# ErickRosete/tacorl

Measured on AMD Instinct MI355X. Metric: offline grad-steps/sec (batch=256, 84x84 RGB), higher is better.
Workload: dtype bf16; 1 GPU; tacorl actor-critic training_step, frozen LMP (BASELINE configs[1]); per_gpu_batch=256, global_batch=256, window=16, image=84x84x3, frames=fp32 CHW (reference batch schema), latent_plan=16, n_action_samples=4, phase=Q (epoch>=bc_epochs), action_decoder_loss=every step (reference behaviour), parallelism=dp1, hip_graph=True, losses_finite=True

## Files before the change

### tacorl_amd/csrc/dense_ops.hip

```cpp
#include <stdio.h>
#include <stdlib.h>
#include <string.h>

#include <type_traits>

#include "../../include/tacorl_hip.h"
#include "enc_bwd_fused.h"
#include "mlp_fused.h"
#include "functors.h"

static thread_local char g_err[256] = "";
#define FAIL(code, ...)                        \
  do {                                         \
    snprintf(g_err, sizeof(g_err), __VA_ARGS__); \
    return (code);                             \
  } while (0)
#define CHECK(x)            \
  do {                      \
    int _r = (x);           \
    if (_r != TACORL_OK) return _r; \
  } while (0)

extern "C" const char* tacorl_hip_last_error(void) { return g_err; }
extern "C" int tacorl_hip_version(void) { return 1; }
// ... 737 lines not shown
  size_t scratch_bytes, fcwt_off[EBW_MAXP], fcwt_each, slab_off, slab_bytes, conv_off, total;
  long so[EBW_MAXP][6], ao[EBW_MAXP][5], sbase[EBW_MAXP];
  long maxn;
};
static const int kFcActs[2] = {ACT_RELU, ACT_NONE};
static bool enc_bwd_plan(int nprob, const int* n_img, int H, int W, EncBwdPlan& pl) {
  if (!enc_dims(H, W, pl.d) || !ebw_supported(H, W) || nprob < 1 || nprob > EBW_MAXP) return false;
  tacorl_encoder_param_layout(pl.po);
  long tot = 0;
  pl.maxn = 0;
  for (int p = 0; p < nprob; p++) {
    pl.sbase[p] = tot;
    tot += enc_bwd_scratch_layout(n_img[p], pl.d, pl.so[p]);
    tacorl_encoder_act_layout(n_img[p], H, W, pl.ao[p]);
    pl.maxn = n_img[p] > pl.maxn ? n_img[p] : pl.maxn;
  }
  size_t b = ((size_t)tot * sizeof(float) + 255) & ~(size_t)255;
  pl.scratch_bytes = b;
  pl.fcwt_each = (mlp_fused_wt_elems(2, kFcDims, nullptr) * 2 + 255) & ~(size_t)255;
  for (int p = 0; p < nprob; p++) { pl.fcwt_off[p] = b; b += pl.fcwt_each; }
  pl.slab_off = b;
  pl.slab_bytes = enc_fc_slab_bytes(nprob, pl.maxn);
  b += pl.slab_bytes;
  pl.conv_off = b;
  pl.total = b + ebw_ws_bytes(nprob, n_img, H, W);
  return true;
}
extern "C" size_t tacorl_encoder_bwd_fused_ws_bytes(int nprob, const int* n_img, int H, int W) {
  EncBwdPlan pl;
  return enc_bwd_plan(nprob, n_img, H, W, pl) ? pl.total : 0;
}
static void enc_bwd_conv_problems(int nprob, const void* const* img, const float* const* params, const float* const* act,
                                  float* const* grads, const int* n_img, const EncBwdPlan& pl, void* ws, EbwProblem* pr) {
  for (int p = 0; p < nprob; p++) {
    const float* P = params[p];
    float* G = grads ? grads[p] : nullptr;
    float* sc = (float*)ws + pl.sbase[p];
    pr[p].img = img ? img[p] : nullptr;
    pr[p].y1 = act ? act[p] + pl.ao[p][0] : nullptr; pr[p].y2 = act ? act[p] + pl.ao[p][1] : nullptr;
    pr[p].dz3 = sc + pl.so[p][2];
    pr[p].w2 = P + pl.po[E_W2]; pr[p].w3 = P + pl.po[E_W3];
    pr[p].g_w1 = G ? G + pl.po[E_W1] : nullptr; pr[p].g_b1 = G ? G + pl.po[E_B1] : nullptr;
    pr[p].g_w2 = G ? G + pl.po[E_W2] : nullptr; pr[p].g_b2 = G ? G + pl.po[E_B2] : nullptr;
    pr[p].g_w3 = G ? G + pl.po[E_W3] : nullptr; pr[p].g_b3 = G ? G + pl.po[E_B3] : nullptr;
    pr[p].n = n_img[p];
  }
}
static int enc_bwd_fc_chain(int nprob, const float* const* params, const float* const* act, const float* const* d_out,
                            const int* n_img, const EncBwdPlan& pl, void* ws, hipStream_t st, int mode) {
  long wo[2], bo[2], src[MF_MAXP * MF_MAXL], dzo[MF_MAXP * MF_MAXL];
  tacorl_mlp_param_layout(2, kFcDims, wo, bo);
  const float* fcp[EBW_MAXP];
  float *dz[EBW_MAXP], *dsa[EBW_MAXP];
  void* wt[EBW_MAXP];
  for (int p = 0; p < nprob; p++) {
    fcp[p] = params[p] + pl.po[E_FW1];
    src[p * MF_MAXL + 0] = pl.ao[p][4];
    src[p * MF_MAXL + 1] = -1;
    dzo[p * MF_MAXL + 0] = pl.sbase[p] + pl.so[p][0];
    dz[p] = (float*)ws;
    dsa[p] = (float*)ws + pl.sbase[p] + pl.so[p][1];
    wt[p] = (unsigned char*)ws + pl.fcwt_off[p];
  }
  return mlp_fused_bwd(nprob, fcp, act, d_out, 32, dz, dsa, 128, wt, n_img, 2, kFcDims, kFcActs, src, dzo, wo, st, mode);
}

extern "C" int tacorl_encoder_bwd_fused_pack(int nprob, const float* const* params, const int* n_img, int H, int W,
                                             void* ws, size_t ws_bytes, tacorl_stream_t stream) {
  EncBwdPlan pl;
  if (!enc_bwd_plan(nprob, n_img, H, W, pl)) FAIL(TACORL_EINVAL, "encoder_bwd_fused_pack: geometry %dx%d / nprob %d", H, W, nprob);
  if (ws_bytes < pl.total) FAIL(TACORL_ENOMEM, "encoder_bwd_fused_pack: workspace too small");
  EbwProblem pr[EBW_MAXP];
  enc_bwd_conv_problems(nprob, nullptr, params, nullptr, nullptr, n_img, pl, ws, pr);
  int rc = enc_bwd_fc_chain(nprob, params, nullptr, nullptr, n_img, pl, ws, (hipStream_t)stream, 1);
  if (rc == TACORL_OK) rc = ebw_conv_backward(nprob, pr, H, W, 0, (unsigned char*)ws + pl.conv_off, pl.total - pl.conv_off, (hipStream_t)stream, 1);
  if (rc != TACORL_OK) FAIL(rc, "encoder_bwd_fused_pack: launch failed (%d)", rc);
  return TACORL_OK;
}
extern "C" int tacorl_encoder_bwd_fused_head(int nprob, const float* const* params, const float* const* act,
                                             const float* const* d_out, const int* n_img, int H, int W, int prepacked,
                                             void* ws, size_t ws_bytes, tacorl_stream_t stream) {
  EncBwdPlan pl;
  if (!enc_bwd_plan(nprob, n_img, H, W, pl)) FAIL(TACORL_EINVAL, "encoder_bwd_fused_head: geometry %dx%d / nprob %d", H, W, nprob);
  if (ws_bytes < pl.total) FAIL(TACORL_ENOMEM, "encoder_bwd_fused_head: workspace too small");
  const int rc = enc_bwd_fc_chain(nprob, params, act, d_out, n_img, pl, ws, (hipStream_t)stream, prepacked ? 2 : 0);
  if (rc != TACORL_OK) FAIL(rc, "encoder_bwd_fused_head: launch failed (%d)", rc);
  return TACORL_OK;
}
extern "C" int tacorl_encoder_bwd_fused_fc_wgrad(int nprob, const float* const* act, const float* const* d_out,
                                                 float* const* grads, const int* n_img, int H, int W, int accumulate,
                                                 void* ws, size_t ws_bytes, tacorl_stream_t stream) {
  hipStream_t st = (hipStream_t)stream;
  EncBwdPlan pl;
  if (!enc_bwd_plan(nprob, n_img, H, W, pl)) FAIL(TACORL_EINVAL, "encoder_bwd_fused_fc_wgrad: geometry %dx%d / nprob %d", H, W, nprob);
  if (ws_bytes < pl.total) FAIL(TACORL_ENOMEM, "encoder_bwd_fused_fc_wgrad: workspace too small");
  const float *sa[EBW_MAXP], *h1[EBW_MAXP], *d_h1[EBW_MAXP];
  float *g_fw1[EBW_MAXP], *g_fb1[EBW_MAXP], *g_fw2[EBW_MAXP], *g_fb2[EBW_MAXP];
  for (int p = 0; p < nprob; p++) {
    sa[p] = act[p] + pl.ao[p][3]; h1[p] = act[p] + pl.ao[p][4];
    d_h1[p] = (const float*)ws + pl.sbase[p] + pl.so[p][0];
    float* G = grads[p];
    g_fw1[p] = G + pl.po[E_FW1]; g_fb1[p] = G + pl.po[E_FB1]; g_fw2[p] = G + pl.po[E_FW2]; g_fb2[p] = G + pl.po[E_FB2];
  }
  void* slab = (unsigned char*)ws + pl.slab_off;
  if (mlp_fused_wgrad_ok(nprob, 2, kFcDims) &&
      mlp_fused_wgrad_slab_floats(nprob, n_img, 2, kFcDims) * sizeof(float) <= pl.slab_bytes) {
    long yoffs[MF_MAXP * MF_MAXL] = {}, dzoffs[MF_MAXP * MF_MAXL] = {};
    const float* dzb[EBW_MAXP];
    for (int p = 0; p < nprob; p++) {
      yoffs[p * MF_MAXL] = pl.ao[p][4];
      dzoffs[p * MF_MAXL] = pl.sbase[p] + pl.so[p][0];
      dzb[p] = (const float*)ws;
    }
    const long wo[2] = {pl.po[E_FW1], pl.po[E_FW2]}, bo[2] = {pl.po[E_FB1], pl.po[E_FB2]};
    if (mlp_fused_wgrad(nprob, sa, 128, act, d_out, 32, dzb, grads, (float*)slab, n_img, 2, kFcDims, yoffs, dzoffs, wo, bo,
                        accumulate, st))
      FAIL(TACORL_ELAUNCH, "encoder_bwd_fused_fc_wgrad: launch failed");
    return TACORL_OK;
  }
  CHECK(k_linear_wgrad(nprob, h1, 256, d_out, 32, n_img, 256, 32, g_fw2, g_fb2, accumulate, slab, pl.slab_bytes, TACORL_BF16, st));
  CHECK(k_linear_wgrad(nprob, sa, 128, d_h1, 256, n_img, 128, 256, g_fw1, g_fb1, accumulate, slab, pl.slab_bytes, TACORL_BF16, st));
  return TACORL_OK;
}
extern "C" int tacorl_encoder_bwd_fused_conv(int nprob, const void* const* img, const float* const* params,
                                             const float* const* act, float* const* grads, const int* n_img, int H, int W,
                                             int accumulate, int prepacked, void* ws, size_t ws_bytes,
                                             tacorl_stream_t stream) {
  return tacorl_encoder_bwd_fused_conv_parts(nprob, img, params, act, grads, n_img, H, W, accumulate, prepacked, 127, ws,
                                             ws_bytes, stream);
}
extern "C" int tacorl_encoder_bwd_fused_conv_parts(int nprob, const void* const* img, const float* const* params,
                                                   const float* const* act, float* const* grads, const int* n_img, int H,
                                                   int W, int accumulate, int prepacked, int parts, void* ws,
                                                   size_t ws_bytes, tacorl_stream_t stream) {
  hipStream_t st = (hipStream_t)stream;
  EncBwdPlan pl;
  if (!enc_bwd_plan(nprob, n_img, H, W, pl)) FAIL(TACORL_EINVAL, "encoder_bwd_fused_conv: geometry %dx%d / nprob %d", H, W, nprob);
  if (ws_bytes < pl.total) FAIL(TACORL_ENOMEM, "encoder_bwd_fused_conv: workspace too small");
  if (pl.d.c3.OH * pl.d.c3.OW > 4 * SAB_MAXI_HUGE) FAIL(TACORL_EINVAL, "encoder_bwd_fused: conv3 output too large");
  if ((parts & EBW_ALL) && (parts & EBW_ALL) != EBW_ALL && !prepacked)
    FAIL(TACORL_EINVAL, "encoder_bwd_fused_conv_parts: partial calls need prepacked fragments");
  EbwProblem pr[EBW_MAXP];
  enc_bwd_conv_problems(nprob, img, params, act, grads, n_img, pl, ws, pr);
  SabArgs sb{};
  for (int p = 0; p < nprob; p++) {
    float* sc = (float*)ws + pl.sbase[p];
    sb.y3[p] = act[p] + pl.ao[p][2]; sb.temp[p] = params[p] + pl.po[E_T]; sb.sa[p] = act[p] + pl.ao[p][3];
    sb.d_sa[p] = sc + pl.so[p][1]; sb.dz3[p] = sc + pl.so[p][2]; sb.dtp[p] = sc + pl.so[p][5];
    sb.gtemp[p] = grads[p] + pl.po[E_T]; sb.n[p] = n_img[p];
  }
  const char* fe = getenv("TACORL_EBW_FUSE3");
  const int fuse3 = fe ? atoi(fe) : 1;
  const bool fused3 = fuse3 && (parts & 127) == 127 && ebw_fused3_supported(H, W);
  if (fused3) {
    for (int p = 0; p < nprob; p++) {
      pr[p].y3 = sb.y3[p]; pr[p].temp = sb.temp[p]; pr[p].sa = sb.sa[p]; pr[p].d_sa = sb.d_sa[p];
      pr[p].dtp = sb.dtp[p]; pr[p].g_temp = sb.gtemp[p];
    }
  }
  if (pl.maxn > 0 && (parts & 1) && !fused3) {
    const int P3 = pl.d.c3.OH * pl.d.c3.OW;
    if (P3 <= 4 * 13) hipLaunchKernelGGL(softargmax_bwd_batch_kernel<13>, dim3((unsigned)pl.maxn, nprob), dim3(256), 0, st, sb, P3, pl.d.c3.OW);
    else if (P3 <= 4 * SAB_MAXI_BIG) hipLaunchKernelGGL(softargmax_bwd_batch_kernel<SAB_MAXI_BIG>, dim3((unsigned)pl.maxn, nprob), dim3(256), 0, st, sb, P3, pl.d.c3.OW);
    else hipLaunchKernelGGL(softargmax_bwd_batch_kernel<SAB_MAXI_HUGE>, dim3((unsigned)pl.maxn, nprob), dim3(256), 0, st, sb, P3, pl.d.c3.OW);
    hipLaunchKernelGGL(sum_to_scalar_batch_kernel, dim3(nprob), dim3(256), 0, st, sb, accumulate);
  }
  if (!(parts & EBW_ALL)) return hipGetLastError() == hipSuccess ? TACORL_OK : TACORL_ELAUNCH;
  const int rc = ebw_conv_backward(nprob, pr, H, W, accumulate, (unsigned char*)ws + pl.conv_off, pl.total - pl.conv_off, st, prepacked ? 2 : 0,
                                   (parts & EBW_ALL) | (fused3 ? EBW_FUSED3 : 0));
  if (rc != TACORL_OK) FAIL(rc, "encoder_bwd_fused_conv: conv backward launch failed (%d)", rc);
  return hipGetLastError() == hipSuccess ? TACORL_OK : TACORL_ELAUNCH;
}
extern "C" int tacorl_encoder_bwd_fused(int nprob, const void* const* img, const float* const* params,
                                        const float* const* act, const float* const* d_out, float* const* grads,
                                        const int* n_img, int H, int W, int accumulate, void* ws, size_t ws_bytes,
                                        tacorl_stream_t stream) {
  int rc = tacorl_encoder_bwd_fused_head(nprob, params, act, d_out, n_img, H, W, 0, ws, ws_bytes, stream);
  if (rc == TACORL_OK) rc = tacorl_encoder_bwd_fused_fc_wgrad(nprob, act, d_out, grads, n_img, H, W, accumulate, ws, ws_bytes, stream);
  if (rc == TACORL_OK) rc = tacorl_encoder_bwd_fused_conv(nprob, img, params, act, grads, n_img, H, W, accumulate, 0, ws, ws_bytes, stream);
  return rc;
}

extern "C" long tacorl_mlp_param_layout(int L, const int* dims, long* w_off, long* b_off) {
  long off = 0;
  for (int l = 0; l < L; l++) {
    if (w_off) w_off[l] = off;
    off = al4(off + (long)dims[l + 1] * dims[l]);
    if (b_off) b_off[l] = off;
    off = al4(off + dims[l + 1]);
  }
  return off;
}
extern "C" long tacorl_mlp_act_layout(int M, int L, const int* dims, const int* acts, long* z_off, long* y_off) {
  long off = 0;
  for (int l = 0; l < L; l++) {
    if (z_off) z_off[l] = -1;
    if (acts[l] == ACT_SILU) { if (z_off) z_off[l] = off; off = al4(off + (long)M * dims[l + 1]); }
    if (y_off) y_off[l] = off;
    off = al4(off + (long)M * dims[l + 1]);
  }
  return off;
}
#define MLP_MAXL 8

struct OutActTbl { const float* d[GEMM_MAXP]; const float* y[GEMM_MAXP]; float* dz[GEMM_MAXP]; int M[GEMM_MAXP]; };
__global__ __launch_bounds__(256) void out_act_grad_kernel(OutActTbl t, int ldo, int N, int act) {
  const int p = blockIdx.y;
  const long total = (long)t.M[p] * N;
  for (long e = (long)blockIdx.x * 256 + threadIdx.x; e < total; e += (long)gridDim.x * 256) {
    const long m = e / N;
    t.dz[p][e] = t.d[p][m * ldo + (e - m * N)] * act_grad(act, t.y[p][e]);
  }
}
static int out_act_grad(int nprob, const OutActTbl& t, int ldo, int N, int act, hipStream_t st) {
  long mx = 0;
  for (int p = 0; p < nprob; p++) mx = (long)t.M[p] * N > mx ? (long)t.M[p] * N : mx;
  if (mx == 0) return TACORL_OK;
  const int gx = cdiv(mx, 256) > 1024 ? 1024 : cdiv(mx, 256);
  hipLaunchKernelGGL(out_act_grad_kernel, dim3(gx, nprob), dim3(256), 0, st, t, ldo, N, act);
  return hipGetLastError() == hipSuccess ? TACORL_OK : TACORL_ELAUNCH;
}

extern "C" int tacorl_mlp_fwd(int nprob, const float* const* x, int ldx, const float* const* params,
                              float* const* act, const int* M, int L, const int* dims, const int* acts, int cd,
                              tacorl_stream_t stream) {
  hipStream_t st = (hipStream_t)stream;
  if (L < 1 || L > MLP_MAXL || nprob < 1 || nprob > GEMM_MAXP) FAIL(TACORL_EINVAL, "mlp_fwd: bad L/nprob");
  long wo[MLP_MAXL], bo[MLP_MAXL];
  tacorl_mlp_param_layout(L, dims, wo, bo);
  for (int l = 0; l < L; l++) {
    const float *xin[GEMM_MAXP], *w[GEMM_MAXP], *b[GEMM_MAXP];
    float *y[GEMM_MAXP], *z[GEMM_MAXP];
    for (int p = 0; p < nprob; p++) {
      long zo[MLP_MAXL], yo[MLP_MAXL];
      tacorl_mlp_act_layout(M[p], L, dims, acts, zo, yo);
      xin[p] = l == 0 ? x[p] : act[p] + yo[l - 1];
      w[p] = params[p] + wo[l]; b[p] = params[p] + bo[l];
      y[p] = act[p] + yo[l]; z[p] = zo[l] >= 0 ? act[p] + zo[l] : nullptr;
    }
    CHECK(k_linear_fwd(nprob, xin, l == 0 ? ldx : dims[l], w, b, y, z, M, dims[l], dims[l + 1], dims[l + 1], acts[l], cd, st));
  }
  return TACORL_OK;
}

extern "C" int tacorl_mlp_fwd_fused_supported(int nprob, int L, const int* dims, int ldx) {
  return mlp_fused_fwd_ok(nprob, L, dims, ldx) ? 1 : 0;
}
extern "C" int tacorl_mlp_lean_supported(int nprob, int L, const int* dims, int ldx, int ldo, int ldd) {
  return mlp_fused_fwd_ok(nprob, L, dims, ldx) && mlp_fused_bwd_ok(nprob, L, dims, ldo, ldd) && mlp_fused_wgrad_ok(nprob, L, dims) ? 1 : 0;
}
static int mlp_fwd_fused_impl(int nprob, const float* const* x, int ldx, const float* const* params,
                              const void* const* params_bf16, float* const* act, const int* M, int L,
                              const int* dims, const int* acts, int lean, tacorl_stream_t stream, const MlpXGather* gather) {
  if (!mlp_fused_fwd_ok(nprob, L, dims, ldx)) FAIL(TACORL_EINVAL, "mlp_fwd_fused: shapes not supported");
  for (int p = 0; p < nprob; p++)
    if (!aligned16(params[p]) || ((uintptr_t)params_bf16[p] & 7) || (!gather && !aligned16(x[p])))
      FAIL(TACORL_EINVAL, "mlp_fwd_fused: problem %d: misaligned pointer", p);
  long wo[MLP_MAXL], bo[MLP_MAXL];
  tacorl_mlp_param_layout(L, dims, wo, bo);
  const float *xs[2][MF_MAXP], *ps[2][MF_MAXP];
  const void* pb[2][MF_MAXP];
  float* as[2][MF_MAXP];
  int Ms[2][MF_MAXP], gm[2][MF_MAXP], n[2] = {0, 0};
  long zo[MF_MAXP * MF_MAXL], yo[MF_MAXP * MF_MAXL], ybf[MF_MAXP * MF_MAXL], sbf[MF_MAXP * MF_MAXL], yout[MF_MAXP];
  for (int p = 0; p < nprob; p++) {
    long z1[MLP_MAXL], y1[MLP_MAXL];
    tacorl_mlp_act_layout(M[p], L, dims, acts, z1, y1);
    const int b = (lean && mlp_big_prob_ok(M[p], L, dims, acts)) ? 1 : 0, q = n[b]++;
    gm[b][q] = p;
    if (gather && gather->xb[p] && (!b || M[p] >= 16384 || !aligned16(gather->xb[p])))
      FAIL(TACORL_EINVAL, "mlp_fwd_fused_gather_xb: problem %d: the bf16 input rows are written only for a lean site's problems of "
                          "2048 .. 16383 rows, 16-byte aligned", p);
    xs[b][q] = x ? x[p] : nullptr; ps[b][q] = params[p]; pb[b][q] = params_bf16[p]; as[b][q] = act[p]; Ms[b][q] = M[p];
    for (int l = 0; l < L; l++) {
      if (b) { ybf[q * MF_MAXL + l] = y1[l]; sbf[q * MF_MAXL + l] = z1[l]; }
      else {
        zo[q * MF_MAXL + l] = z1[l];
        yo[q * MF_MAXL + l] = (lean && l + 1 < L && z1[l] >= 0) ? -1 : y1[l];
      }
    }
    if (b) yout[q] = y1[L - 1];
  }
  if (n[1]) {
    const int rc = mlp_big_fwd(n[1], xs[1], ldx, ps[1], pb[1], as[1], Ms[1], L, dims, acts, ybf, sbf, yout, wo, bo, (hipStream_t)stream, gather, gm[1]);
    if (rc != TACORL_OK) FAIL(rc, "mlp_fwd_fused: many-row launch failed (%d)", rc);
  }
  if (n[0]) {
    const int rc = mlp_fused_fwd(n[0], xs[0], ldx, ps[0], pb[0], as[0], Ms[0], L, dims, acts, zo, yo, wo, bo, (hipStream_t)stream, gather, gm[0]);
    if (rc != TACORL_OK) FAIL(rc, "mlp_fwd_fused: launch failed (%d)", rc);
  }
  return TACORL_OK;
}
extern "C" int tacorl_mlp_fwd_fused(int nprob, const float* const* x, int ldx, const float* const* params,
                                    const void* const* params_bf16, float* const* act, const int* M, int L,
                                    const int* dims, const int* acts, int lean, tacorl_stream_t stream) {
  return mlp_fwd_fused_impl(nprob, x, ldx, params, params_bf16, act, M, L, dims, acts, lean, stream, nullptr);
}
extern "C" int tacorl_mlp_fwd_fused_gather_supported(int nprob, const int* M, int L, const int* dims, const int* acts, int ldx,
                                                     int lean) {
  (void)M; (void)acts; (void)lean;
  return mlp_fused_fwd_ok(nprob, L, dims, ldx) ? 1 : 0;
}
namespace {
struct XbWritten { const void* ptr; int M; };
thread_local XbWritten g_xb_written[16];
thread_local int g_xb_next = 0;
void xb_note(const void* ptr, int M) {
  for (XbWritten& e : g_xb_written)
    if (e.ptr == ptr) { e.M = M; return; }
  g_xb_written[g_xb_next] = XbWritten{ptr, M};
  g_xb_next = (g_xb_next + 1) % 16;
}
bool xb_noted(const void* ptr, int M) {
  for (const XbWritten& e : g_xb_written)
    if (e.ptr == ptr && e.M == M) return true;
  return false;
}
void xb_forget(const void* ptr) {
  for (XbWritten& e : g_xb_written)
    if (e.ptr == ptr) e = XbWritten{nullptr, 0};
}
}
// ... 335 lines not shown
```

### tacorl_amd/csrc/enc_bwd_fused.h

```cpp
#pragma once
#include <hip/hip_runtime.h>
#include <stddef.h>

#define EBW_MAXP 8

struct EbwProblem {
  const void* img;
  const void* y1;
  const void* y2;
  const float* dz3;
  const float* w2;
  const float* w3;
  float *g_w1, *g_b1, *g_w2, *g_b2, *g_w3, *g_b3;
  int n;
  const float *y3, *temp, *sa, *d_sa;
  float *dtp, *g_temp;
};

bool ebw_supported(int H, int W);
size_t ebw_ws_bytes(int nprob, const int* n_img, int H, int W);
enum { EBW_DGRAD3 = 2, EBW_WGRAD3 = 4, EBW_DGRAD2 = 8, EBW_WGRAD2 = 16, EBW_WGRAD1 = 32, EBW_REDUCE = 64, EBW_ALL = 126,
       EBW_FUSED3 = 128 };
bool ebw_fused3_supported(int H, int W);
int ebw_conv_backward(int nprob, const EbwProblem* pr, int H, int W, int accumulate, void* ws, size_t ws_bytes,
                      hipStream_t st, int mode, int parts = EBW_ALL);
```

### tacorl_amd/csrc/encoder_bwd_fused.hip

```cpp
#include "enc_bwd_fused.h"

#include <stdlib.h>

#include <type_traits>

#include "common.h"

namespace {

constexpr int NT = 512;
constexpr int NW = NT / 64;

constexpr int cmax(int a, int b) { return a > b ? a : b; }
constexpr int pitch8(int need) { return (need % 16 <= 8) ? need - need % 16 + 8 : need - need % 16 + 24; }

template <int KH_, int S_, int CI_, int CO_, int IH_, int IW_>
struct ConvL {
  static constexpr int KH = KH_, KW = KH_, S = S_, CI = CI_, CO = CO_, IH = IH_, IW = IW_;
  static constexpr int OH = (IH - KH) / S + 1, OW = (IW - KW) / S + 1;
  static constexpr int PH = (IH + S - 1) / S, PW = (IW + S - 1) / S;
  static constexpr int KA = KH / S, KB = KW / S;
  static constexpr int TAPS = KH * KW * CI;
  static constexpr int NPL = CI * S * S;
  static constexpr int PWP = (PW + 7) / 8 * 8;
// ... 622 lines not shown
      float v[G::K3];
#pragma unroll
      for (int k = 0; k < G::K3; k++) v[k] = vn[k];
      const float gx = gn[0], gy = gn[1], dot = gn[0] * fn[0] + gn[1] * fn[1];
      asm volatile("" : : "v"(gx), "v"(gy), "v"(dot) : "memory");
#pragma unroll
      for (int k = 0; k < G::K3; k++) asm volatile("" : : "v"(v[k]) : "memory");
      if (nxt < n_img) { fetch(nxt); fetch3(nxt); }
      const __bf16* yb = y2s + kb * G::Y2E;
      float mx = -INFINITY;
#pragma unroll
      for (int k = 0; k < G::K3; k++) {
        v[k] *= it;
        if (wl + NW3 * k < G::P3) mx = fmaxf(mx, v[k]);
      }
      float se = 0.f;
#pragma unroll
      for (int k = 0; k < G::K3; k++) se += (wl + NW3 * k < G::P3) ? __expf(v[k] - mx) : 0.f;
      shm[wl * 64 + lane] = mx;
      shs[wl * 64 + lane] = se;
      __syncthreads();
      {
        float mw[NW3], sw[NW3];
#pragma unroll
        for (int ww = 0; ww < NW3; ww++) { mw[ww] = shm[ww * 64 + lane]; sw[ww] = shs[ww * 64 + lane]; }
        __builtin_amdgcn_sched_barrier(0);
#pragma unroll
        for (int ww = 0; ww < NW3; ww++) mx = fmaxf(mx, mw[ww]);
        se = 0.f;
#pragma unroll
        for (int ww = 0; ww < NW3; ww++) se += sw[ww] * __expf(mw[ww] - mx);
      }
      const float rse = 1.0f / se;
#pragma unroll
      for (int k = 0; k < G::K3; k++) {
        const int i = wl + NW3 * k;
        if (i < G::P3) {
          const int iy = i / L::OW;
          const float pr = __expf(v[k] - mx) * rse;
          const float ds = pr * (gx * (float)(i - iy * L::OW) + gy * (float)iy - dot);
          dt -= ds * v[k] * it;
          dzh[((iy + L::HA) * L::C + (i - iy * L::OW) + L::HB) * L::PP + lane] = (__bf16)(v[k] != 0.f ? ds * it : 0.f);
        }
      }
      if (img != j0) flush(img - a.wpp, z2s + (kb ^ 1) * G::Z2E);
      __syncthreads();
      if constexpr (ROLE == 0) {
        __bf16* zw = z2s + kb * G::Z2E;
#pragma unroll
        for (int tg = 0; tg < NGRP3; tg++) {
          f32x4 o[TG3];
#pragma unroll
          for (int u = 0; u < TG3; u++) o[u] = f32x4{0.f, 0.f, 0.f, 0.f};
          constexpr int HK = L::KS / 2;
          static_assert(L::KS % 2 == 0, "fragment steps in two halves");
          auto aoff = [&](int ks) {
            const int tp = ks / (L::CO / 32), hf = ks % (L::CO / 32), ta = tp / L::KB, tb = tp % L::KB;
            return ((L::HA - ta) * L::C + L::HB - tb) * L::PP + 32 * hf;
          };
          bf16x8 A[TG3][HK];
#pragma unroll
          for (int ks = 0; ks < HK; ks++)
#pragma unroll
            for (int u = 0; u < TG3; u++)
              A[u][ks] = *reinterpret_cast<const bf16x8*>(dzh + abase[tg * TG3 + u < MT ? tg * TG3 + u : MT - 1] + aoff(ks));
          __builtin_amdgcn_sched_barrier(0);
#pragma unroll
          for (int ks = 0; ks < L::KS; ks++) {
#pragma unroll
            for (int u = 0; u < TG3; u++) {
              o[u] = __builtin_amdgcn_mfma_f32_16x16x32_bf16(Bf[ks], A[u][ks % HK], o[u], 0, 0, 0);
              if (ks + HK < L::KS)
                A[u][ks % HK] = *reinterpret_cast<const bf16x8*>(dzh + abase[tg * TG3 + u < MT ? tg * TG3 + u : MT - 1] + aoff(ks + HK));
            }
            __builtin_amdgcn_sched_barrier(0);
          }
#pragma unroll
          for (int u = 0; u < TG3; u++) {
            const int t = tg * TG3 + u;
            if (t >= MT) continue;
            const int oi = obase + t * 16 * L::CI;
            if (oi < L::PH * L::PW * L::CI) {
              const uint2 yv = *reinterpret_cast<const uint2*>(yb + (oi >> 6) * G::CIP + (oi & 63));
              const bool m0 = (((yv.x & 0xffffu) - 1u) & 0xffffu) < 0x7fffu, m1 = (((yv.x >> 16) - 1u) & 0xffffu) < 0x7fffu;
              const bool m2 = (((yv.y & 0xffffu) - 1u) & 0xffffu) < 0x7fffu, m3 = (((yv.y >> 16) - 1u) & 0xffffu) < 0x7fffu;
              *reinterpret_cast<bf16x4*>(zw + oi) =
                  bf16x4{(__bf16)(m0 ? o[u][0] : 0.f), (__bf16)(m1 ? o[u][1] : 0.f), (__bf16)(m2 ? o[u][2] : 0.f),
                         (__bf16)(m3 ? o[u][3] : 0.f)};
            }
          }
        }
      } else {
#pragma unroll
        for (int s = 0; s < G::KS; s++) {
          constexpr int JB = (G::NPW + 2) / 3;
          bf16x8 A[G::MPW], B[JB];
#pragma unroll
          for (int i = 0; i < G::MPW; i++) {
            const int col = 16 * (mg * G::MPW + i) + 4 * pc;
            A[i] = tr_frag(dzh + zr0[s] + col, dzh + zr1[s] + col);
          }
#pragma unroll
          for (int jb = 0; jb < G::NPW; jb += JB) {
#pragma unroll
            for (int j = jb; j < jb + JB && j < G::NPW; j++) {
              const int tofs = ((j / L::KW) * L::IW + j % L::KW) * G::CIP;
              B[j - jb] = tr_frag(yb + ir0[s] + coff + tofs, yb + ir1[s] + coff + tofs);
            }
            __builtin_amdgcn_sched_barrier(0);
#pragma unroll
            for (int j = jb; j < jb + JB && j < G::NPW; j++)
#pragma unroll
              for (int i = 0; i < G::MPW; i++) acc[i][j] = __builtin_amdgcn_mfma_f32_16x16x32_bf16(A[i], B[j - jb], acc[i][j], 0, 0, 0);
            __builtin_amdgcn_sched_barrier(0);
          }
          if (ng == 0) {
#pragma unroll
            for (int i = 0; i < G::MPW; i++) bacc[i] = __builtin_amdgcn_mfma_f32_16x16x32_bf16(A[i], ones, bacc[i], 0, 0, 0);
          }
        }
      }
      if (nxt < n_img) put(y2s + (kb ^ 1) * G::Y2E);
      __syncthreads();
    }
    if (j0 < n_img) flush(j0 + ((n_img - 1 - j0) / a.wpp) * a.wpp, z2s + (kb ^ 1) * G::Z2E);
    if constexpr (ROLE == 1) {
      float* sl = a.slab + (long)blockIdx.x * TG::SLABF;
#pragma unroll
      for (int i = 0; i < G::MPW; i++)
#pragma unroll
        for (int j = 0; j < G::NPW; j++)
          *reinterpret_cast<f32x4*>(sl + (((wv * G::MPW + i) * G::NPW + j) * 64 + lane) * 4) = acc[i][j];
      if (ng == 0 && l16 == 0) {
#pragma unroll
        for (int i = 0; i < G::MPW; i++)
#pragma unroll
          for (int r = 0; r < 4; r++) sl[L::CO * L::TAPS + 16 * (mg * G::MPW + i) + 4 * g + r] = bacc[i][r];
      }
    }
    dt = wave_sum(dt);
    if (lane == 0) shd[w] = dt;
    __syncthreads();
    if (tid == 0 && j0 < n_img) {
      float sum = 0.f;
#pragma unroll
      for (int ww = 0; ww < NW3; ww++) sum += shd[ww];
      a.dtp[p][j0] = sum;
    }
  };
  if (w < ND3) run(std::integral_constant<int, 0>{});
  else run(std::integral_constant<int, 1>{});
}

inline size_t al256(size_t x) { return (x + 255) & ~(size_t)255; }
inline int cdivi(long a, long b) { return (int)((a + b - 1) / b); }
constexpr int cdivi_c(int a, int b) { return (a + b - 1) / b; }

struct WsPlan {
  size_t wpk2[EBW_MAXP], wpk3[EBW_MAXP], dz2[EBW_MAXP], dz1[EBW_MAXP], slab1, slab2, slab3, total;
  int wpp;
};
template <class G>
WsPlan plan(int nprob, const int* n) {
  WsPlan w{};
  long maxn = 1;
  for (int p = 0; p < nprob; p++) maxn = n[p] > maxn ? n[p] : maxn;
  const int per = 256 / nprob > 1 ? 256 / nprob : 1;
  w.wpp = (int)(per < maxn ? per : maxn);
  size_t off = 0;
  for (int p = 0; p < nprob; p++) {
    w.wpk2[p] = off; off += al256((size_t)G::L2::NCOMBO * G::L2::KS * 64 * 16);
    w.wpk3[p] = off; off += al256((size_t)G::L3::NCOMBO * G::L3::KS * 64 * 16);
    w.dz2[p] = off; off += al256((size_t)n[p] * G::L3::IH * G::L3::IW * 64 * 2);
    w.dz1[p] = off; off += al256((size_t)n[p] * G::L2::IH * G::L2::IW * 32 * 2);
  }
  const size_t nwg = (size_t)nprob * w.wpp;
  w.slab1 = off; off += al256(nwg * TrGeo<typename G::L1>::SLABF * 4);
  w.slab2 = off; off += al256(nwg * TrGeo<typename G::L2>::SLABF * 4);
  w.slab3 = off; off += al256(nwg * TrGeo<typename G::L3>::SLABF * 4);
  w.total = off;
  return w;
}

template <class K>
int set_lds(K kern, size_t bytes) {
  return hipFuncSetAttribute(reinterpret_cast<const void*>(kern), hipFuncAttributeMaxDynamicSharedMemorySize, (int)bytes) ==
                 hipSuccess ? 0 : -1;
}

template <class L, class InT, class DzT>
int launch_wgrad_tr(const WgArgs& a, int nwg, hipStream_t st) {
  auto kern = ebw_wgrad_tr_kernel<L, InT, DzT>;
  constexpr size_t lds = TrGeo<L>::lds_bytes;
  static int once = set_lds(kern, lds);
  if (once) return TACORL_ELAUNCH;
  hipLaunchKernelGGL(kern, dim3(nwg), dim3(NT), lds, st, a);
  return TACORL_OK;
}
template <class L, class DzT>
int launch_dgrad(const DgArgs& a, int nwg, hipStream_t st) {
  auto kern = ebw_dgrad_kernel<L, DzT>;
  constexpr size_t lds = dgrad_lds_bytes<L>();
  static int once = set_lds(kern, lds);
  if (once) return TACORL_ELAUNCH;
  hipLaunchKernelGGL(kern, dim3(nwg), dim3(NT), lds, st, a);
  return TACORL_OK;
}
template <class L>
int launch_l3(const L3Args& a, int nwg, hipStream_t st) {
  auto kern = ebw_l3_kernel<L>;
  constexpr size_t lds = L3Geo<L>::lds_bytes;
  static int once = set_lds(kern, lds);
  if (once) return TACORL_ELAUNCH;
  hipLaunchKernelGGL(kern, dim3(nwg), dim3(NT3), lds, st, a);
  return TACORL_OK;
}
template <class G>
int run(int nprob, const EbwProblem* pr, int accumulate, void* ws, size_t ws_bytes, hipStream_t st, int mode, int parts) {
  using L1 = typename G::L1; using L2 = typename G::L2; using L3 = typename G::L3;
  int n[EBW_MAXP];
  for (int p = 0; p < nprob; p++) n[p] = pr[p].n;
  const WsPlan w = plan<G>(nprob, n);
  if (ws_bytes < w.total) return TACORL_ENOMEM;
  unsigned char* base = (unsigned char*)ws;
  const int nwg = nprob * w.wpp;
  PkArgs k2{}, k3{};
  for (int p = 0; p < nprob; p++) {
    k2.w[p] = pr[p].w2; k2.out[p] = (uint4*)(base + w.wpk2[p]);
    k3.w[p] = pr[p].w3; k3.out[p] = (uint4*)(base + w.wpk3[p]);
  }
  if (mode != 2) {
    hipLaunchKernelGGL((ebw_pack2_kernel<L2, L3>), dim3(cdivi(L2::NCOMBO * L2::KS * 64, 256) + cdivi(L3::NCOMBO * L3::KS * 64, 256), nprob),
                       dim3(256), 0, st, k2, k3);
  }
  if (mode == 1) return hipGetLastError() == hipSuccess ? TACORL_OK : TACORL_ELAUNCH;
  DgArgs d3{}, d2{};
  WgArgs g3{}, g2{}, g1{};
  float *gw1[EBW_MAXP], *gb1[EBW_MAXP], *gw2[EBW_MAXP], *gb2[EBW_MAXP], *gw3[EBW_MAXP], *gb3[EBW_MAXP];
  for (int p = 0; p < nprob; p++) {
    __bf16* dz2 = (__bf16*)(base + w.dz2[p]);
    __bf16* dz1 = (__bf16*)(base + w.dz1[p]);
    d3.dz[p] = pr[p].dz3; d3.yin[p] = (const __bf16*)pr[p].y2; d3.wpk[p] = k3.out[p]; d3.dx[p] = dz2; d3.n[p] = n[p];
    d2.dz[p] = dz2; d2.yin[p] = (const __bf16*)pr[p].y1; d2.wpk[p] = k2.out[p]; d2.dx[p] = dz1; d2.n[p] = n[p];
    g3.in[p] = pr[p].y2; g3.dz[p] = pr[p].dz3; g3.n[p] = n[p];
    g2.in[p] = pr[p].y1; g2.dz[p] = dz2; g2.n[p] = n[p];
    g1.in[p] = pr[p].img; g1.dz[p] = dz1; g1.n[p] = n[p];
    gw1[p] = pr[p].g_w1; gb1[p] = pr[p].g_b1; gw2[p] = pr[p].g_w2; gb2[p] = pr[p].g_b2;
    gw3[p] = pr[p].g_w3; gb3[p] = pr[p].g_b3;
  }
  d3.wpp = d2.wpp = g3.wpp = g2.wpp = g1.wpp = w.wpp;
  constexpr int dg2 = 2;
  long maxn = 1;
  for (int p = 0; p < nprob; p++) maxn = n[p] > maxn ? n[p] : maxn;
  auto per_cu = [](size_t lds) { return (size_t)dg2 * lds <= 160 * 1024 ? dg2 : 1; };
  const int k3w = per_cu(dgrad_lds_bytes<L3>()), k2w = per_cu(dgrad_lds_bytes<L2>());
  d3.wpp = (int)((long)k3w * w.wpp < maxn ? (long)k3w * w.wpp : maxn);
  d2.wpp = (int)((long)k2w * w.wpp < maxn ? (long)k2w * w.wpp : maxn);
  g1.slab = (float*)(base + w.slab1); g2.slab = (float*)(base + w.slab2); g3.slab = (float*)(base + w.slab3);
  int rc;
  const bool fused3 = (parts & EBW_FUSED3) != 0;
  if (fused3 && (parts & EBW_ALL) != EBW_ALL) return TACORL_EINVAL;
  {
    if (fused3) {
      L3Args f{};
      for (int p = 0; p < nprob; p++) {
        f.y3[p] = pr[p].y3; f.temp[p] = pr[p].temp; f.sa[p] = pr[p].sa; f.d_sa[p] = pr[p].d_sa;
        f.y2[p] = (const __bf16*)pr[p].y2; f.wpk[p] = k3.out[p]; f.dz2[p] = (__bf16*)(base + w.dz2[p]);
        f.dtp[p] = pr[p].dtp; f.n[p] = n[p];
      }
      f.slab = g3.slab; f.wpp = w.wpp;
      if constexpr (L3Geo<L3>::ok) {
        if ((rc = launch_l3<L3>(f, nwg, st))) return rc;
      } else {
        return TACORL_EINVAL;
      }
    } else {
      if ((parts & EBW_DGRAD3) && (rc = launch_dgrad<L3, float>(d3, nprob * d3.wpp, st))) return rc;
      if ((parts & EBW_WGRAD3) && (rc = launch_wgrad_tr<L3, __bf16, float>(g3, nwg, st))) return rc;
    }
    if ((parts & EBW_DGRAD2) && (rc = launch_dgrad<L2, __bf16>(d2, nprob * d2.wpp, st))) return rc;
    if ((parts & EBW_WGRAD2) && (rc = launch_wgrad_tr<L2, __bf16, __bf16>(g2, nwg, st))) return rc;
    if ((parts & EBW_WGRAD1) && (rc = launch_wgrad_tr<L1, __bf16, __bf16>(g1, nwg, st))) return rc;
    if (!(parts & EBW_REDUCE)) return hipGetLastError() == hipSuccess ? TACORL_OK : TACORL_ELAUNCH;
    RdTrArgs t{};
    t.slab[0] = g1.slab; t.slab[1] = g2.slab; t.slab[2] = g3.slab;
    auto fill = [&](int l, auto geo, int co, int taps) {
      using TG = decltype(geo);
      t.co[l] = co; t.taps[l] = taps; t.mpw[l] = TG::MPW; t.npw[l] = TG::NPW; t.mgrp[l] = TG::T::MGRP;
      t.ngrp[l] = TG::T::NGRP; t.kgrp[l] = TG::T::KGRP; t.slabf[l] = TG::SLABF;
    };
    fill(0, TrGeo<L1>{}, L1::CO, L1::TAPS); fill(1, TrGeo<L2>{}, L2::CO, L2::TAPS); fill(2, TrGeo<L3>{}, L3::CO, L3::TAPS);
    t.wpp = w.wpp; t.accumulate = accumulate;
    for (int p = 0; p < nprob; p++) {
      t.gw[0][p] = gw1[p]; t.gb[0][p] = gb1[p]; t.gw[1][p] = gw2[p]; t.gb[1][p] = gb2[p];
      t.gw[2][p] = gw3[p]; t.gb[2][p] = gb3[p];
    }
    constexpr int maxper_t = cmax(L1::SLABF, cmax(L2::SLABF, L3::SLABF));
    static_assert(cdivi_c(maxper_t, 64) - 1 > cdivi_c(L1::SLABF, 64), "the temperature block must lie beyond conv1's elements");
    if (fused3) {
      for (int p = 0; p < nprob; p++) { t.dtp[p] = pr[p].dtp; t.g_temp[p] = pr[p].g_temp; t.ndt[p] = n[p] < w.wpp ? n[p] : w.wpp; }
      t.ileave[2] = 1; t.mpw[2] = L3Geo<L3>::MPW; t.npw[2] = L3Geo<L3>::NPW; t.mgrp[2] = L3Tile::MGRP; t.ngrp[2] = L3Tile::NGRP;
    }
    hipLaunchKernelGGL(ebw_reduce_tr_kernel, dim3(cdivi(maxper_t, 64), 3 * nprob), dim3(256), 0, st, t);
    return hipGetLastError() == hipSuccess ? TACORL_OK : TACORL_ELAUNCH;
  }
}

}

#define EBW_GEOMS(X) X(84, 84) X(64, 64) X(44, 60) X(128, 128) X(150, 200)

bool ebw_fused3_supported(int H, int W) {
#define X(h, w) if (H == h && W == w) return L3Geo<Geo<h, w>::L3>::ok;
  EBW_GEOMS(X)
#undef X
  return false;
}
bool ebw_supported(int H, int W) {
#define X(h, w) if (H == h && W == w) return true;
  EBW_GEOMS(X)
#undef X
  return false;
}
size_t ebw_ws_bytes(int nprob, const int* n_img, int H, int W) {
  if (nprob < 1 || nprob > EBW_MAXP) return 0;
#define X(h, w) if (H == h && W == w) return plan<Geo<h, w>>(nprob, n_img).total;
  EBW_GEOMS(X)
#undef X
  return 0;
}
int ebw_conv_backward(int nprob, const EbwProblem* pr, int H, int W, int accumulate, void* ws, size_t ws_bytes,
                      hipStream_t st, int mode, int parts) {
  if (nprob < 1 || nprob > EBW_MAXP) return TACORL_EINVAL;
#define X(h, w) if (H == h && W == w) return run<Geo<h, w>>(nprob, pr, accumulate, ws, ws_bytes, st, mode, parts);
  EBW_GEOMS(X)
#undef X
  return TACORL_EINVAL;
}
```

Baseline: 1368 grad-steps/s.

## Fuse conv2 dgrad and wgrad into one warp-specialized backward kernel

Adds a fused conv2 backward kernel in which some waves compute the data gradient, applying the ReLU mask from y1, while the other waves compute weight and bias gradients. Both read the same double-buffered LDS copy of dz2 and y1. It replaces two separate launches, each re-reading dz2 from global memory, and is enabled by default whenever conv3 fusion is active and the geometry supports it. The cost is heavy LDS use per workgroup (double buffer of halo plus y1 image), which may lower occupancy, and a new reduction tiling layout for conv2.

Measured after the change: 1375 grad-steps/s, median of 2. No clear change (+0.5%).

```diff
diff --git a/tacorl_amd/csrc/dense_ops.hip b/tacorl_amd/csrc/dense_ops.hip
--- a/tacorl_amd/csrc/dense_ops.hip
+++ b/tacorl_amd/csrc/dense_ops.hip
@@ -913,6 +913,7 @@
   const char* fe = getenv("TACORL_EBW_FUSE3");
   const int fuse3 = fe ? atoi(fe) : 1;
   const bool fused3 = fuse3 && (parts & 127) == 127 && ebw_fused3_supported(H, W);
+  const bool fused2 = fused3 && ebw_fused2_supported(H, W);
   if (fused3) {
     for (int p = 0; p < nprob; p++) {
       pr[p].y3 = sb.y3[p]; pr[p].temp = sb.temp[p]; pr[p].sa = sb.sa[p]; pr[p].d_sa = sb.d_sa[p];
@@ -928,7 +929,7 @@
   }
   if (!(parts & EBW_ALL)) return hipGetLastError() == hipSuccess ? TACORL_OK : TACORL_ELAUNCH;
   const int rc = ebw_conv_backward(nprob, pr, H, W, accumulate, (unsigned char*)ws + pl.conv_off, pl.total - pl.conv_off, st, prepacked ? 2 : 0,
-                                   (parts & EBW_ALL) | (fused3 ? EBW_FUSED3 : 0));
+                                   (parts & EBW_ALL) | (fused3 ? EBW_FUSED3 : 0) | (fused2 ? EBW_FUSED2 : 0));
   if (rc != TACORL_OK) FAIL(rc, "encoder_bwd_fused_conv: conv backward launch failed (%d)", rc);
   return hipGetLastError() == hipSuccess ? TACORL_OK : TACORL_ELAUNCH;
 }
diff --git a/tacorl_amd/csrc/enc_bwd_fused.h b/tacorl_amd/csrc/enc_bwd_fused.h
--- a/tacorl_amd/csrc/enc_bwd_fused.h
+++ b/tacorl_amd/csrc/enc_bwd_fused.h
@@ -20,7 +20,9 @@
 bool ebw_supported(int H, int W);
 size_t ebw_ws_bytes(int nprob, const int* n_img, int H, int W);
 enum { EBW_DGRAD3 = 2, EBW_WGRAD3 = 4, EBW_DGRAD2 = 8, EBW_WGRAD2 = 16, EBW_WGRAD1 = 32, EBW_REDUCE = 64, EBW_ALL = 126,
-       EBW_FUSED3 = 128 };
+       EBW_FUSED3 = 128,
+       EBW_FUSED2 = 256 };
 bool ebw_fused3_supported(int H, int W);
+bool ebw_fused2_supported(int H, int W);
 int ebw_conv_backward(int nprob, const EbwProblem* pr, int H, int W, int accumulate, void* ws, size_t ws_bytes,
                       hipStream_t st, int mode, int parts = EBW_ALL);
diff --git a/tacorl_amd/csrc/encoder_bwd_fused.hip b/tacorl_amd/csrc/encoder_bwd_fused.hip
--- a/tacorl_amd/csrc/encoder_bwd_fused.hip
+++ b/tacorl_amd/csrc/encoder_bwd_fused.hip
@@ -798,6 +798,220 @@
   else run(std::integral_constant<int, 1>{});
 }
 
+struct L2Args {
+  const __bf16* dz[EBW_MAXP];
+  const __bf16* y1[EBW_MAXP];
+  const uint4* wpk[EBW_MAXP];
+  __bf16* dx[EBW_MAXP];
+  float* slab;
+  int n[EBW_MAXP];
+  int wpp;
+};
+struct L2Tile { static constexpr int MGRP = 1, NGRP = 4, KGRP = 1; };
+template <class L>
+struct L2Geo {
+  using TG = TrGeo<L>;
+  static constexpr int NPIX = L::OH * L::OW, KS = (NPIX + 31) / 32;
+  static constexpr int HALO = L::R * L::C * L::PP;
+  static constexpr int CIP = TG::CIP, Y1E = (L::IH * L::IW * CIP + 7) / 8 * 8;
+  static constexpr int BUF_EL = HALO + Y1E;
+  static constexpr int MPW = L::MT / L2Tile::MGRP, NPW = L::NTL / L2Tile::NGRP;
+  static constexpr size_t lds_bytes = (size_t)2 * BUF_EL * 2;
+  static_assert(L::PP == TG::DZR && HALO % 8 == 0, "the halo image's pixel pitch is the transposing read's row pitch");
+  static constexpr bool ok = L::S == 2 && L::CI == 32 && L::CO == 64 && L::NCLS == NW3 - ND3 && KS <= 4 && lds_bytes <= 160 * 1024;
+};
+
+template <class L>
+__global__ __launch_bounds__(NT3) void ebw_l2_kernel(L2Args a) {
+  using G = L2Geo<L>;
+  using T = L2Tile;
+  static_assert(T::MGRP * T::NGRP * T::KGRP == NW3 - ND3, "wgrad waves");
+  static_assert(G::ok, "geometry not supported by the fused conv2 backward");
+  extern __shared__ __attribute__((aligned(16))) unsigned char smem[];
+  __bf16* lds = reinterpret_cast<__bf16*>(smem);
+  const int tid = threadIdx.x, lane = tid & 63, g = lane >> 4, l16 = lane & 15, q = l16 >> 2, pc = l16 & 3;
+  const int w = __builtin_amdgcn_readfirstlane(tid >> 6);
+  const int p = blockIdx.x / a.wpp, j0 = blockIdx.x - p * a.wpp;
+  const int n_img = a.n[p];
+#pragma unroll
+  for (int k = 0; k < 2; k++)
+    for (int e = tid; e < G::HALO / 8; e += NT3) reinterpret_cast<uint4*>(lds + k * G::BUF_EL)[e] = make_uint4(0u, 0u, 0u, 0u);
+  const __bf16* dz = a.dz[p];
+  const __bf16* y1 = a.y1[p];
+  constexpr int NTR = ND3 * 64;
+  constexpr int NCG = L::CO / 8, NCH = G::NPIX * NCG, CPT = (NCH + NTR - 1) / NTR;
+  constexpr int YCG = L::CI / 8, NYC = L::IH * L::IW * YCG, CPY = (NYC + NTR - 1) / NTR;
+  auto run = [&](auto role_tag) {
+    constexpr int ROLE = decltype(role_tag)::value;
+    bf16x8 pre[ROLE == 0 ? CPT : 1], ypre[ROLE == 0 ? CPY : 1];
+    auto fetch = [&](int img) {
+      if constexpr (ROLE == 0) {
+#pragma unroll
+        for (int r = 0; r < CPT; r++) {
+          const int c = tid + r * NTR;
+          pre[r] = *reinterpret_cast<const bf16x8*>(dz + (long)img * G::NPIX * L::CO + 8 * (c < NCH ? c : NCH - 1));
+        }
+#pragma unroll
+        for (int r = 0; r < CPY; r++) {
+          const int c = tid + r * NTR;
+          ypre[r] = *reinterpret_cast<const bf16x8*>(y1 + (long)img * L::IH * L::IW * L::CI + 8 * (c < NYC ? c : NYC - 1));
+        }
+      }
+    };
+    auto put = [&](__bf16* buf) {
+      if constexpr (ROLE == 0) {
+#pragma unroll
+        for (int r = 0; r < CPT; r++) {
+          const int c = tid + r * NTR;
+          if (c < NCH) {
+            const int pix = c / NCG, cg = c - pix * NCG, oy = pix / L::OW, ox = pix - oy * L::OW;
+            *reinterpret_cast<bf16x8*>(buf + ((oy + L::HA) * L::C + ox + L::HB) * L::PP + 8 * cg) = pre[r];
+          }
+        }
+        __bf16* yb = buf + G::HALO;
+#pragma unroll
+        for (int r = 0; r < CPY; r++) {
+          const int c = tid + r * NTR;
+          if (c < NYC) *reinterpret_cast<bf16x8*>(yb + (c / YCG) * G::CIP + 8 * (c % YCG)) = ypre[r];
+        }
+      }
+    };
+    constexpr int MT = L::MTC;
+    bf16x8 Bf[ROLE == 0 ? L::NTI : 1][ROLE == 0 ? L::KS : 1];
+    int abase[ROLE == 0 ? MT : 1], oidx[ROLE == 0 ? MT : 1];
+    if constexpr (ROLE == 0) {
+      const int cls = w, py = cls / L::S, px = cls % L::S;
+#pragma unroll
+      for (int nt = 0; nt < L::NTI; nt++)
+#pragma unroll
+        for (int ks = 0; ks < L::KS; ks++)
+          Bf[nt][ks] = __builtin_bit_cast(bf16x8, a.wpk[p][((cls * L::NTI + nt) * L::KS + ks) * 64 + lane]);
+#pragma unroll
+      for (int t = 0; t < MT; t++) {
+        const int m0 = 16 * t + l16;
+        const int m = m0 < L::PH * L::PW ? m0 : L::PH * L::PW - 1;
+        const int Y = m / L::PW, X = m - Y * L::PW;
+        abase[t] = (Y * L::C + X) * L::PP + 8 * g;
+        const int Y0 = m0 / L::PW, X0 = m0 - Y0 * L::PW, y = L::S * Y0 + py, x = L::S * X0 + px;
+        oidx[t] = (m0 < L::PH * L::PW && y < L::IH && x < L::IW) ? (y * L::IW + x) * L::CI + 4 * g : -1;
+      }
+    }
+    static_assert(L::KH == T::NGRP && G::NPW == L::KW * (L::CI / 16), "one kernel row per wave group");
+    const int wv = w - ND3, ng = wv % T::NGRP, mg = (wv / T::NGRP) % T::MGRP;
+    int zr0[ROLE == 1 ? G::KS : 1], zr1[ROLE == 1 ? G::KS : 1], ir0[ROLE == 1 ? G::KS : 1], ir1[ROLE == 1 ? G::KS : 1];
+    f32x4 acc[ROLE == 1 ? G::MPW : 1][ROLE == 1 ? G::NPW : 1], bacc[ROLE == 1 ? G::MPW : 1];
+    bf16x8 ones;
+    if constexpr (ROLE == 1) {
+#pragma unroll
+      for (int s = 0; s < G::KS; s++) {
+        const int P0 = 32 * s + 4 * g + q, P1 = P0 + 16;
+        const int Q0 = P0 < G::NPIX ? P0 : G::NPIX - 1, Q1 = P1 < G::NPIX ? P1 : G::NPIX - 1;
+        zr0[s] = (P0 < G::NPIX ? ((P0 / L::OW + L::HA) * L::C + P0 % L::OW + L::HB) * L::PP : 0) + 4 * pc;
+        zr1[s] = (P1 < G::NPIX ? ((P1 / L::OW + L::HA) * L::C + P1 % L::OW + L::HB) * L::PP : 0) + 4 * pc;
+        ir0[s] = ((Q0 / L::OW) * L::S * L::IW + (Q0 % L::OW) * L::S + ng * L::IW) * G::CIP + 4 * pc;
+        ir1[s] = ((Q1 / L::OW) * L::S * L::IW + (Q1 % L::OW) * L::S + ng * L::IW) * G::CIP + 4 * pc;
+      }
+#pragma unroll
+      for (int i = 0; i < G::MPW; i++) {
+        bacc[i] = f32x4{0.f, 0.f, 0.f, 0.f};
+#pragma unroll
+        for (int j = 0; j < G::NPW; j++) acc[i][j] = f32x4{0.f, 0.f, 0.f, 0.f};
+      }
+#pragma unroll
+      for (int j = 0; j < 8; j++) ones[j] = (__bf16)1.0f;
+    }
+    __syncthreads();
+    if (j0 < n_img) { fetch(j0); put(lds); }
+    if constexpr (ROLE == 0) __builtin_amdgcn_s_waitcnt(0x0f70);
+    __syncthreads();
+    int kb = 0;
+    for (int img = j0; img < n_img; img += a.wpp, kb ^= 1) {
+      const int nxt = img + a.wpp;
+      if (nxt < n_img) fetch(nxt);
+      const __bf16* dzh = lds + kb * G::BUF_EL;
+      const __bf16* yb = dzh + G::HALO;
+      if constexpr (ROLE == 0) {
+        __bf16* dx = a.dx[p] + (long)img * L::IH * L::IW * L::CI;
+#pragma unroll
+        for (int t = 0; t < MT; t++) {
+          f32x4 o[L::NTI];
+#pragma unroll
+          for (int nt = 0; nt < L::NTI; nt++) o[nt] = f32x4{0.f, 0.f, 0.f, 0.f};
+          bf16x8 A[L::KS];
+#pragma unroll
+          for (int ks = 0; ks < L::KS; ks++) {
+            const int tp = ks / (L::CO / 32), hf = ks % (L::CO / 32), ta = tp / L::KB, tb = tp % L::KB;
+            A[ks] = *reinterpret_cast<const bf16x8*>(dzh + abase[t] + ((L::HA - ta) * L::C + L::HB - tb) * L::PP + 32 * hf);
+          }
+#pragma unroll
+          for (int ks = 0; ks < L::KS; ks++)
+#pragma unroll
+            for (int nt = 0; nt < L::NTI; nt++) o[nt] = __builtin_amdgcn_mfma_f32_16x16x32_bf16(Bf[nt][ks], A[ks], o[nt], 0, 0, 0);
+          if (oidx[t] >= 0) {
+#pragma unroll
+            for (int nt = 0; nt < L::NTI; nt++) {
+              const int oi = oidx[t] + 16 * nt;
+              const uint2 yv = *reinterpret_cast<const uint2*>(yb + (oi / L::CI) * G::CIP + (oi % L::CI));
+              const bool m0 = (((yv.x & 0xffffu) - 1u) & 0xffffu) < 0x7fffu, m1 = (((yv.x >> 16) - 1u) & 0xffffu) < 0x7fffu;
+              const bool m2 = (((yv.y & 0xffffu) - 1u) & 0xffffu) < 0x7fffu, m3 = (((yv.y >> 16) - 1u) & 0xffffu) < 0x7fffu;
+              *reinterpret_cast<bf16x4*>(dx + oi) =
+                  bf16x4{(__bf16)(m0 ? o[nt][0] : 0.f), (__bf16)(m1 ? o[nt][1] : 0.f), (__bf16)(m2 ? o[nt][2] : 0.f),
+                         (__bf16)(m3 ? o[nt][3] : 0.f)};
+            }
+          }
+        }
+      } else {
+#pragma unroll
+        for (int s = 0; s < G::KS; s++) {
+          constexpr int JB = (G::NPW + 1) / 2;
+          bf16x8 A[G::MPW], B[JB];
+#pragma unroll
+          for (int i = 0; i < G::MPW; i++) {
+            const int col = 16 * (mg * G::MPW + i);
+            A[i] = tr_frag(dzh + zr0[s] + col, dzh + zr1[s] + col);
+          }
+#pragma unroll
+          for (int jb = 0; jb < G::NPW; jb += JB) {
+#pragma unroll
+            for (int j = jb; j < jb + JB && j < G::NPW; j++) {
+              const int tofs = (j / (L::CI / 16)) * G::CIP + 16 * (j % (L::CI / 16));
+              B[j - jb] = tr_frag(yb + ir0[s] + tofs, yb + ir1[s] + tofs);
+            }
+            __builtin_amdgcn_sched_barrier(0);
+#pragma unroll
+            for (int j = jb; j < jb + JB && j < G::NPW; j++)
+#pragma unroll
+              for (int i = 0; i < G::MPW; i++) acc[i][j] = __builtin_amdgcn_mfma_f32_16x16x32_bf16(A[i], B[j - jb], acc[i][j], 0, 0, 0);
+            __builtin_amdgcn_sched_barrier(0);
+          }
+          if (ng == 0) {
+#pragma unroll
+            for (int i = 0; i < G::MPW; i++) bacc[i] = __builtin_amdgcn_mfma_f32_16x16x32_bf16(A[i], ones, bacc[i], 0, 0, 0);
+          }
+        }
+      }
+      if (nxt < n_img) put(lds + (kb ^ 1) * G::BUF_EL);
+      __syncthreads();
+    }
+    if constexpr (ROLE == 1) {
+      float* sl = a.slab + (long)blockIdx.x * G::TG::SLABF;
+#pragma unroll
+      for (int i = 0; i < G::MPW; i++)
+#pragma unroll
+        for (int j = 0; j < G::NPW; j++)
+          *reinterpret_cast<f32x4*>(sl + (((wv * G::MPW + i) * G::NPW + j) * 64 + lane) * 4) = acc[i][j];
+      if (ng == 0 && l16 == 0) {
+#pragma unroll
+        for (int i = 0; i < G::MPW; i++)
+#pragma unroll
+          for (int r = 0; r < 4; r++) sl[L::CO * L::TAPS + 16 * (mg * G::MPW + i) + 4 * g + r] = bacc[i][r];
+      }
+    }
+  };
+  if (w < ND3) run(std::integral_constant<int, 0>{});
+  else run(std::integral_constant<int, 1>{});
+}
+
 inline size_t al256(size_t x) { return (x + 255) & ~(size_t)255; }
 inline int cdivi(long a, long b) { return (int)((a + b - 1) / b); }
 constexpr int cdivi_c(int a, int b) { return (a + b - 1) / b; }
@@ -861,6 +1075,15 @@
   hipLaunchKernelGGL(kern, dim3(nwg), dim3(NT3), lds, st, a);
   return TACORL_OK;
 }
+template <class L>
+int launch_l2(const L2Args& a, int nwg, hipStream_t st) {
+  auto kern = ebw_l2_kernel<L>;
+  constexpr size_t lds = L2Geo<L>::lds_bytes;
+  static int once = set_lds(kern, lds);
+  if (once) return TACORL_ELAUNCH;
+  hipLaunchKernelGGL(kern, dim3(nwg), dim3(NT3), lds, st, a);
+  return TACORL_OK;
+}
 template <class G>
 int run(int nprob, const EbwProblem* pr, int accumulate, void* ws, size_t ws_bytes, hipStream_t st, int mode, int parts) {
   using L1 = typename G::L1; using L2 = typename G::L2; using L3 = typename G::L3;
@@ -905,7 +1128,8 @@
   g1.slab = (float*)(base + w.slab1); g2.slab = (float*)(base + w.slab2); g3.slab = (float*)(base + w.slab3);
   int rc;
   const bool fused3 = (parts & EBW_FUSED3) != 0;
-  if (fused3 && (parts & EBW_ALL) != EBW_ALL) return TACORL_EINVAL;
+  const bool fused2 = (parts & EBW_FUSED2) != 0;
+  if ((fused3 || fused2) && (parts & EBW_ALL) != EBW_ALL) return TACORL_EINVAL;
   {
     if (fused3) {
       L3Args f{};
@@ -924,8 +1148,22 @@
       if ((parts & EBW_DGRAD3) && (rc = launch_dgrad<L3, float>(d3, nprob * d3.wpp, st))) return rc;
       if ((parts & EBW_WGRAD3) && (rc = launch_wgrad_tr<L3, __bf16, float>(g3, nwg, st))) return rc;
     }
-    if ((parts & EBW_DGRAD2) && (rc = launch_dgrad<L2, __bf16>(d2, nprob * d2.wpp, st))) return rc;
-    if ((parts & EBW_WGRAD2) && (rc = launch_wgrad_tr<L2, __bf16, __bf16>(g2, nwg, st))) return rc;
+    if (fused2) {
+      L2Args f{};
+      for (int p = 0; p < nprob; p++) {
+        f.dz[p] = (const __bf16*)(base + w.dz2[p]); f.y1[p] = (const __bf16*)pr[p].y1; f.wpk[p] = k2.out[p];
+        f.dx[p] = (__bf16*)(base + w.dz1[p]); f.n[p] = n[p];
+      }
+      f.slab = g2.slab; f.wpp = w.wpp;
+      if constexpr (L2Geo<L2>::ok) {
+        if ((rc = launch_l2<L2>(f, nwg, st))) return rc;
+      } else {
+        return TACORL_EINVAL;
+      }
+    } else {
+      if ((parts & EBW_DGRAD2) && (rc = launch_dgrad<L2, __bf16>(d2, nprob * d2.wpp, st))) return rc;
+      if ((parts & EBW_WGRAD2) && (rc = launch_wgrad_tr<L2, __bf16, __bf16>(g2, nwg, st))) return rc;
+    }
     if ((parts & EBW_WGRAD1) && (rc = launch_wgrad_tr<L1, __bf16, __bf16>(g1, nwg, st))) return rc;
     if (!(parts & EBW_REDUCE)) return hipGetLastError() == hipSuccess ? TACORL_OK : TACORL_ELAUNCH;
     RdTrArgs t{};
@@ -947,6 +1185,9 @@
       for (int p = 0; p < nprob; p++) { t.dtp[p] = pr[p].dtp; t.g_temp[p] = pr[p].g_temp; t.ndt[p] = n[p] < w.wpp ? n[p] : w.wpp; }
       t.ileave[2] = 1; t.mpw[2] = L3Geo<L3>::MPW; t.npw[2] = L3Geo<L3>::NPW; t.mgrp[2] = L3Tile::MGRP; t.ngrp[2] = L3Tile::NGRP;
     }
+    if (fused2) {
+      t.mpw[1] = L2Geo<L2>::MPW; t.npw[1] = L2Geo<L2>::NPW; t.mgrp[1] = L2Tile::MGRP; t.ngrp[1] = L2Tile::NGRP;
+    }
     hipLaunchKernelGGL(ebw_reduce_tr_kernel, dim3(cdivi(maxper_t, 64), 3 * nprob), dim3(256), 0, st, t);
     return hipGetLastError() == hipSuccess ? TACORL_OK : TACORL_ELAUNCH;
   }
@@ -958,6 +1199,12 @@
 
 bool ebw_fused3_supported(int H, int W) {
 #define X(h, w) if (H == h && W == w) return L3Geo<Geo<h, w>::L3>::ok;
+  EBW_GEOMS(X)
+#undef X
+  return false;
+}
+bool ebw_fused2_supported(int H, int W) {
+#define X(h, w) if (H == h && W == w) return L2Geo<Geo<h, w>::L2>::ok;
   EBW_GEOMS(X)
 #undef X
   return false;
```
